# cwitkowitz/amt-tools

Measured on AMD Instinct MI355X. Metric: audio frames/sec (OnsetsFrames+Mel-229 inference), higher is better.
Workload: dtype bf16

## Files before the change

amt_tools_amd/_lib.py:

```python
import ctypes as C
import os
import re

_HERE = os.path.dirname(os.path.abspath(__file__))
LIB_PATH = os.environ.get('AMTX_LIB_PATH') or os.path.join(_HERE, 'csrc', 'libamtx.so')
HEADER_PATH = os.path.join(os.path.dirname(_HERE), 'include', 'amtx.h')

_lib = None


class AmtxError(RuntimeError):
    pass


ERR_UNSUPPORTED = -3


def declared_symbols():
    with open(HEADER_PATH) as f:
        text = f.read()
    text = re.sub(r'/\*.*?\*/', '', text, flags=re.S)
    return sorted(set(re.findall(r'\b(amtx_[a-z0-9_]+)\s*\(', text)))


# ... 11 lines not shown
    'amtx_spec_num_frames': (_L, [_P, _L]),
    'amtx_spec_filterbank': (_I, [_P, _P]),
    'amtx_spec_power': (_I, [_P, _P, _L, _L, _I, _P, _P, _P]),
    'amtx_spec_scale': (_I, [_P, _P, _P, _P, _I, _L, _I, _I, _P, _P]),
    'amtx_of_model_create': (_I, [C.POINTER(_P), _I, _I, _I, _I, _I, _I]),
    'amtx_has_f16': (_I, []),
    'amtx_of_model_destroy': (_I, [_P]),
    'amtx_of_model_set_tensor': (_I, [_P, C.c_char_p, _P, _L]),
    'amtx_of_model_finalize': (_I, [_P]),
    'amtx_of_model_set_tensor_device': (_I, [_P, C.c_char_p, _P, _L]),
    'amtx_of_model_finalize_device': (_I, [_P, _P]),
    'amtx_of_workspace_bytes': (C.c_size_t, [_P, _I, _I]),
    'amtx_of_forward': (_I, [_P, _P, _L, _L, _L, _L, _I, _I, _P, C.c_size_t, _P, _P, _P, _P, _P, _P]),
    'amtx_of_fuses_db_scale': (_I, [_P]),
    'amtx_of_conv_stack_fused': (_I, [_P, _I, _I]),
    'amtx_of_forward_power': (_I, [_P, _P, _L, _L, _L, _P, _P, _I, _I, _P, C.c_size_t, _P, _P, _P, _P, _P, _P]),
    'amtx_of_takes_feats16': (_I, [_P]),
    'amtx_of_forward_feats16': (_I, [_P, _P, _I, _I, _P, C.c_size_t, _P, _P, _P, _P, _P, _P]),
    'amtx_of_offsets': (_I, [_P, _P, C.c_size_t, _I, _I, _P, _P, _P]),
    'amtx_of_num_stages': (_I, []),
    'amtx_of_stage_name': (C.c_char_p, [_I]),
    'amtx_of_profile_enable': (_I, [_P, _I]),
    'amtx_of_profile_read': (_I, [_P, C.POINTER(C.c_double), C.POINTER(_I)]),
    'amtx_linear_packed_elems': (_L, [_I, _I, _I]),
    'amtx_linear_pack': (_I, [_P, _I, _I, _I, _P]),
    'amtx_linear_fwd': (_I, [_P, _L, _I, _P, _I, _P, _P, _L, _I, _L, _I, _I, _P]),
    'amtx_split_planes': (_I, [_P, _L, _I, _P, _I, _L, _L, _P]),
    'amtx_linear_fwd_split': (_I, [_P, _L, _L, _P, _P, _P, _L, _I, _L, _L, _I, _I, _P]),
    'amtx_conv3x3_packed_elems': (_L, [_I, _I]),
    'amtx_conv3x3_pack': (_I, [_P, _P, _I, _I, _P]),
# ... 130 lines not shown
```

amt_tools_amd/csrc/amtx_f16_names.h:

```cpp
#pragma once
#ifdef AMTX_F16
#define amtx_conv3x3_wfrag_elems amtx_conv3x3_wfrag_elems_f16
#define amtx_conv3x3_pack_host amtx_conv3x3_pack_host_f16
#define amtx_conv1_wfrag_elems amtx_conv1_wfrag_elems_f16
#define amtx_conv1_pack_host amtx_conv1_pack_host_f16
#define amtx_launch_conv3x3 amtx_launch_conv3x3_f16
#define amtx_launch_conv1 amtx_launch_conv1_f16
#define amtxdbg_conv_prof amtxdbg_conv_prof_f16
#define amtx_conv_stack_fused_ok amtx_conv_stack_fused_ok_f16
#define amtx_launch_conv_stack amtx_launch_conv_stack_f16
#define amtxdbg_convf_prof amtxdbg_convf_prof_f16
#define amtx_conv3x3_gen_ntc amtx_conv3x3_gen_ntc_f16
#define amtx_conv3x3_gen_wfrag_elems amtx_conv3x3_gen_wfrag_elems_f16
#define amtx_conv3x3_gen_pack_host amtx_conv3x3_gen_pack_host_f16
#define amtx_conv1g_wfrag_elems amtx_conv1g_wfrag_elems_f16
#define amtx_conv1g_pack_host amtx_conv1g_pack_host_f16
#define amtx_conv3x3_gen_can_fuse1 amtx_conv3x3_gen_can_fuse1_f16
#define amtx_launch_conv3x3_gen amtx_launch_conv3x3_gen_f16
#define amtxdbg_convg_prof amtxdbg_convg_prof_f16
#define amtx_pack_bn_fold_dev amtx_pack_bn_fold_dev_f16
#define amtx_pack_conv3x3_dev amtx_pack_conv3x3_dev_f16
#define amtx_pack_conv1_dev amtx_pack_conv1_dev_f16
#define amtx_pack_conv_gen_dev amtx_pack_conv_gen_dev_f16
#define amtx_pack_conv1g_dev amtx_pack_conv1g_dev_f16
#define amtx_pack_scale_rows_dev amtx_pack_scale_rows_dev_f16
// ... 19 lines not shown
```

amt_tools_amd/csrc/amtx_kernels.h:

```cpp
#pragma once
#include "amtx_common.h"

enum { AMTX_T_BF16 = 0, AMTX_T_F32 = 1, AMTX_T_SPLIT = 2 };

static inline size_t amtx_tsize(int t) { return t == AMTX_T_BF16 ? 2 : 4; }

struct GemmArgs {
    const void* A; int64_t lda; int a_type;
    const bf16_t* W; int n_pad, k_pad, planes;
    const float* bias;
    void* C; int64_t ldc; int c_type;
    int64_t M; int N, K;
    int groups; int64_t a_gs, w_gs, bias_gs, c_gs;
    const int2* pair_map = nullptr; float* pair_out = nullptr; int64_t pair_gs = 0, pair_pitch = 0;
    int pair_rows[16] = {0, 0, 0, 0, 0, 0, 0, 0, 0, 0, 0, 0, 0, 0, 0, 0};
    float* pair_max = nullptr; int pair_nh = 0;
    float* roll_out = nullptr; int roll_T = 0; float roll_thr = 0.5f; int roll_group = 0;
    bf16_t* copy16 = nullptr; int64_t copy16_ld = 0; int copy16_col0 = 0, copy16_gs = 0, copy16_pad = 0;
    int64_t a_plane = 0;
    int64_t a_valid_lo = 0, a_valid_hi = 0;
    int64_t a_split = 0, c_split = 0;
};
bool amtx_gemm_has_roll_epilogue(const GemmArgs& g);
int amtx_launch_gemm(const GemmArgs& g, hipStream_t stream);
// ... 3 lines not shown
void amtx_gemm_pack_dims(int N, int K, int* n_pad, int* k_pad);
void amtx_gemm_pack_host(const float* W, int64_t ldw, int N, int K, int planes, bf16_t* out);

struct ConvArgs {
    const void* in; int in_type;
    const bf16_t* wfrag; int planes;
    const float* shift;
    void* out; int out_type;
    int B, T, F, c_out;
    int groups; int64_t in_gs, w_gs, shift_gs, out_gs;
    const float* feats = nullptr; int64_t f_stride_b = 0, f_stride_c = 0, f_stride_t = 0, f_stride_f = 0;
    int c_in = 0;
    const bf16_t* w1frag = nullptr; const float* shift1 = nullptr;
    int64_t w1_gs = 0;
    const float* f_clip_max = nullptr; const float* f_ref = nullptr;
    const void* feats16 = nullptr;
    int64_t out_ts = 0;
    int64_t in_split = 0, out_split = 0;
};
int amtx_launch_conv3x3(const ConvArgs& c, hipStream_t stream);
int amtx_launch_convx3(const ConvArgs& c, hipStream_t stream);
int amtx_launch_convx12(const ConvArgs& c, hipStream_t stream);
size_t amtx_conv1_wfrag_elems(int c_in, int planes);
void amtx_conv1_pack_host(const float* w, const float* scale, int c_in, int planes, bf16_t* out);
size_t amtx_conv3x3_wfrag_elems(int c_out, int planes);
void amtx_conv3x3_pack_host(const float* w, const float* scale, int c_out, int planes, bf16_t* out);

bool amtx_conv_stack_fused_ok(int B, int T, int F, int groups);
int amtx_launch_conv_stack(const ConvArgs& c2, const bf16_t* w3frag, int64_t w3_gs, const float* shift3, void* out, int64_t out_gs,
                           int64_t out_plane, hipStream_t stream);

int amtx_conv3x3_gen_ntc(int c_in, int c_out);
size_t amtx_conv3x3_gen_wfrag_elems(int c_in, int c_out, int planes);
void amtx_conv3x3_gen_pack_host(const float* w , const float* scale, int c_in, int c_out, int planes, bf16_t* out);
int amtx_launch_conv3x3_gen(const ConvArgs& c, int c_in, hipStream_t stream);
static inline __host__ __device__ bool amtx_conv1g_tapk(int c_in, int planes) { return (planes == 1 || planes == 2) && c_in >= 2 && c_in <= 8; }
size_t amtx_conv1g_wfrag_elems(int c_in, int c_mid, int planes);
void amtx_conv1g_pack_host(const float* w , const float* scale, int c_in, int c_mid, int planes, bf16_t* out);
bool amtx_conv3x3_gen_can_fuse1(int c_in, int c_mid, int c_out, int planes);

struct Conv1Args {
    const float* in; int64_t stride_b, stride_c, stride_t, stride_f;
    const float* w;
// ... 59 lines not shown
```

amt_tools_amd/csrc/convf.hip:

```cpp

#include "amtx_f16_names.h"
#include "amtx_kernels.h"

#include <algorithm>
#include <cstdlib>

namespace {

constexpr int RT = 4;
constexpr int R2 = 16 * RT;
constexpr int r3_of(bool halo) { return halo ? R2 - 2 : R2 - 4; }
constexpr int r1_of(bool halo) { return halo ? R2 + 2 : R2; }
constexpr int R1A = R2 + 2;
constexpr int RFA = R1A + 2;
constexpr int CS = 8;
constexpr int CP = CS / 2;
constexpr int RC1 = 2 * CS + 2;
constexpr int RC2 = 2 * CP + 2;
constexpr int PITCH1 = RC1 + 1;
constexpr int PITCH2 = RC2 + 1;
constexpr int ROWB1 = PITCH1 * 16, ROWB2 = PITCH2 * 16;
constexpr int PLANE1 = (R1A * ROWB1 + 255) / 256 * 256;
constexpr int PLANE2 = (R2 * ROWB2 + 255) / 256 * 256;
constexpr int A1_OFF = 0;
constexpr int A2_OFF = 4 * PLANE1;
constexpr int SLAB_COLS = CS + 4;
constexpr int SLAB_LOAD = CS + 2;
constexpr int SLABP = SLAB_COLS * 2;
constexpr int SLAB_BYTES = (RFA * SLABP + 15) / 16 * 16;
constexpr int SLAB_OFF = A2_OFF + 4 * PLANE2;
constexpr int SH3_OFF = SLAB_OFF + 3 * SLAB_BYTES + 128 + 1024;
constexpr int W1_OFF = SH3_OFF + 64 * 4;
constexpr int SH1_OFF = W1_OFF + 8 * 1024;
constexpr int LDS_BYTES = SH1_OFF + 32 * 4;
constexpr int FPRE = (RFA * SLAB_LOAD + 255) / 256;
constexpr int XB = CS / 4;
static_assert(LDS_BYTES <= 160 * 1024, "LDS");
static_assert(CP == 4 && XB == 2, "wave roles below are written for 8 layer2 columns per step");

typedef __attribute__((ext_vector_type(8))) __bf16 mfma_bf16x8;
__device__ __forceinline__ f32x4_t mfma16(uint4 a, uint4 b, f32x4_t c) {
    return amtx_mfma_16x16x32(a, b, c);
}
__device__ __forceinline__ void settle(const uint4& v) { asm volatile("" ::"v"(v.x), "v"(v.y), "v"(v.z), "v"(v.w)); }
__device__ __forceinline__ void settle(float v) { asm volatile("" ::"v"(v)); }

#ifdef AMTX_CONVF_TIMING
__device__ unsigned long long g_convf_prof[16];
#define CONVF_TICK(SLOT)                                                   \
    do {                                                                   \
        const unsigned long long now_ = __builtin_readcyclecounter();      \
        prof_acc[SLOT] += now_ - prof_t;                                   \
        prof_t = now_;                                                     \
    } while (0)
#else
#define CONVF_TICK(SLOT) do {} while (0)
#endif
#if defined(AMTX_CONVF_TIMING) || defined(AMTX_CONVF_ABLATE)
#define CONVF_DBG(BIT) ((dbg & (BIT)) != 0)
#else
#define CONVF_DBG(BIT) false
#endif

struct ConvFArgs {
    const float* feats; int64_t f_stride_b, f_stride_t, f_stride_f;
    const float* f_clip_max; const float* f_ref;
    const bf16_t* w1frag; int64_t w1_gs; const float* shift1;
    const bf16_t* w2frag; int64_t w2_gs; const float* shift2;
    const bf16_t* w3frag; int64_t w3_gs; const float* shift3;
    bf16_t* out; int64_t out_gs;
    int64_t out_plane;
    int B, T, F;
};

struct Pos { int kk, j, b, r0; };
template <int R3_>
__device__ __forceinline__ Pos pos_first_t(int first, int ntt) {
    Pos p;
    p.kk = 0; p.j = 0; p.b = first / ntt; p.r0 = (first - p.b * ntt) * R3_;
    return p;
}
template <int R3_>
__device__ __forceinline__ void pos_next_t(Pos& p, int nstep, int ntt) {
    ++p.kk;
    if (++p.j == nstep) {
        p.j = 0;
        p.r0 += R3_;
        if (p.r0 >= ntt * R3_) { p.r0 = 0; ++p.b; }
    }
}

template <bool HALO>
__global__ __launch_bounds__(512, 2) void convf_kernel(ConvFArgs a, int nstep, int ntt, int nstrips, int per_block, int dbg) {
    constexpr int R3 = r3_of(HALO), R1 = r1_of(HALO), RF = R1 + 2;
    constexpr int FITEMS = RF * SLAB_LOAD;
    constexpr int NUNITS = RT * XB + (HALO ? 1 : 0);
    auto pos_first = [](int first_, int ntt_) { return pos_first_t<R3>(first_, ntt_); };
    auto pos_next = [](Pos& p_, int nstep_, int ntt_) { pos_next_t<R3>(p_, nstep_, ntt_); };
    extern __shared__ __attribute__((aligned(16))) char smem[];
    const int tid = threadIdx.x, lane = tid & 63;
    const int wave = __builtin_amdgcn_readfirstlane(tid >> 6);
    const int grp = blockIdx.y;
    const int g = lane >> 4, trow = lane & 15;
    const int first = blockIdx.x * per_block;
    const int mine = min(per_block, nstrips - first);
    if (mine <= 0) return;
    const int K = mine * nstep;
    const int F2 = a.F >> 1, F4 = F2 >> 1;
    const bool db = a.f_clip_max != nullptr;

    typedef short s16x2 __attribute__((ext_vector_type(2)));
#define CONVF_L1_BEGIN(P, U)                                                                                \
        const char* slab = smem + SLAB_OFF + ((P).kk & 1) * SLAB_BYTES;                                     \
        const int base1 = ((P).kk * CS) % RC1;       \
        const int u = (U);                                                                                  \
        const bool mainu = !HALO || u < NUNITS - 1;                                             \
        const int row1 = mainu ? 16 * (u >> 1) + n16 : R2 + (n16 & 1);                                      \
        const int xb = mainu ? (u & 1) : (n16 >> 1);                                                        \
        const char* fp = slab + (row1 + gg) * SLABP + 8 * xb;                                               \
        const uint2 b0 = *reinterpret_cast<const uint2*>(fp);                                               \
        const uint2 b1 = *reinterpret_cast<const uint2*>(fp + 8);                                           \
        const uint4 bh = make_uint4(b0.x, b0.y, b1.x, b1.y);                                                \
         \
            \
        const uint32_t rowmask = ((unsigned)((P).r0 - 2 + row1) < (unsigned)a.T && xb < XB) ? 0xffffffffu : 0u; \
        const int c1l = CS * (P).j - 1 + 4 * xb;                 \
        const int slotl = base1 + 4 * xb;                                                                   \
        const int dst_row = A1_OFF + g1 * PLANE1 + row1 * ROWB1;                                            \
        const int dst_scratch = SLAB_OFF + 2 * SLAB_BYTES + 128 + (lane_o & 63) * 16;                       \
         \
            \
        const int tu_ = (P).r0 - 2 + 16 * (u >> 1), cu_ = CS * (P).j - 1 + 4 * (u & 1);                     \
        const bool lean = mainu && tu_ >= 0 && tu_ + 15 < a.T && cu_ >= 0 && cu_ + 3 < a.F;                 \
        const int slots_ = base1 + 4 * (u & 1);
#define CONVF_L1_STORE_LEAN(Q, ACC0, ACC1)                                                                  \
        do {                                                                                                \
            uint32_t pk[4];                                                                                 \
            pk[0] = pack_bf16x2((ACC0)[0], (ACC0)[1]); pk[1] = pack_bf16x2((ACC0)[2], (ACC0)[3]);           \
            pk[2] = pack_bf16x2((ACC1)[0], (ACC1)[1]); pk[3] = pack_bf16x2((ACC1)[2], (ACC1)[3]);           \
            _Pragma("unroll") for (int h = 0; h < 4; ++h)                                                   \
                pk[h] = __builtin_bit_cast(uint32_t, __builtin_elementwise_max(__builtin_bit_cast(s16x2, pk[h]), (s16x2){0, 0})); \
            int sq = slots_ + (Q);                                                                          \
            sq = sq >= RC1 ? sq - RC1 : sq;                                                                 \
            *reinterpret_cast<uint4*>(smem + dst_row + sq * 16) = make_uint4(pk[0], pk[1], pk[2], pk[3]);   \
// ... 41 lines not shown
                for (int nt = 0; nt < 2; ++nt) settle(w1t[q][nt]);
#pragma unroll
            for (int tap = 0; tap < 9; ++tap)
#pragma unroll
                for (int nt = 0; nt < 2; ++nt) settle(wf[tap][nt]);
#pragma unroll
            for (int nt = 0; nt < 2; ++nt)
#pragma unroll
                for (int r = 0; r < 4; ++r) { settle(sh1[nt][r]); settle(sh2[nt][r]); }
        }
        if constexpr (!HALO) {
            constexpr int per = (R1A - R1) * ROWB1 / 16;
            for (int i = tid; i < 4 * per; i += 256)
                reinterpret_cast<uint4*>(smem + A1_OFF + (i / per) * PLANE1 + R1 * ROWB1)[i % per] = make_uint4(0, 0, 0, 0);
        }
        for (int i = tid; i < 2 * RFA * 2; i += 256) {
            const int s = i / (RFA * 2), r = i % (RFA * 2);
            *reinterpret_cast<uint16_t*>(smem + SLAB_OFF + s * SLAB_BYTES + (r >> 1) * SLABP + (SLAB_LOAD + (r & 1)) * 2) = 0;
        }

        float fpre[FPRE];
        float fown = 0.f, fref = 0.f;
        unsigned fvalid = 0;
        int fcell[FPRE], foff[FPRE], loff[FPRE];
#pragma unroll
        for (int n = 0; n < FPRE; ++n) {
            const int it = tid + 256 * n;
            const int fi = it / SLAB_LOAD, fc = it % SLAB_LOAD;
            fcell[n] = it < FITEMS ? (fi << 8 | fc) : -256;
            foff[n] = it < FITEMS ? fi * (int)a.f_stride_t + fc * (int)a.f_stride_f : 0;
            loff[n] = it < FITEMS ? fi * SLABP + fc * 2 : 2 * SLAB_BYTES + 64 + (tid & 31) * 2;
        }
        const int fst = (int)a.f_stride_t, fsf = (int)a.f_stride_f;
#define CONVF_ISSUE_LOADS(P)                                                                                \
        do {                                                                                                \
            const float* fb = a.feats + (int64_t)(P).b * a.f_stride_b;                                      \
            const int tb = (P).r0 - 3, cb = CS * (P).j - 2;                                                 \
            const int wb = tb * fst + cb * fsf;                  \
            fvalid = 0;                                                                                     \
            _Pragma("unroll") for (int n = 0; n < FPRE; ++n) {                                              \
                const bool ok = (unsigned)(tb + (fcell[n] >> 8)) < (unsigned)a.T && (unsigned)(cb + (fcell[n] & 255)) < (unsigned)a.F; \
                fvalid |= ok ? (1u << n) : 0u;                                                              \
                fpre[n] = fb[(unsigned)(ok ? wb + foff[n] : 0)];                                            \
            }                                                                                               \
            if (db) {    \
                fown = a.f_clip_max[(P).b];                                                                 \
                fref = a.f_ref[(P).b];                                                                      \
            }                                                                                               \
        } while (0)
#define CONVF_WRITE_SLAB(KK)                                                                                \
        do {                                                                                                \
            DbScale dbs = {0.f, 0.f};                                                                       \
            if (db) dbs = db_scale_make(fown, fref);                                                        \
            char* slab = smem + SLAB_OFF + ((KK) & 1) * SLAB_BYTES;                                         \
            _Pragma("unroll") for (int n = 0; n < FPRE; ++n) {                                              \
                float v = fpre[n];                                                                          \
                if (db) v = db_scale_apply(v, dbs);                                                         \
                v = (fvalid >> n) & 1u ? v : 0.f;                                                           \
                *reinterpret_cast<uint16_t*>(slab + loff[n]) = (uint16_t)pack_bf16x2(v, 0.f);               \
            }                                                                                               \
        } while (0)

        const int lane_a2 = A2_OFF + g * PLANE2 + trow * ROWB2;
        const int n16 = trow, g1 = g, gg = min(g, 2), lane_o = lane;
        const int lane_a1 = A1_OFF + g * PLANE1 + trow * ROWB1;
#define CONVF_L1_PUNIT(P, U)                                                                                \
        do {                                                                                                \
            CONVF_L1_BEGIN(P, U)                                                                            \
            f32x4_t acc1[4][2];                                                                             \
            _Pragma("unroll") for (int q = 0; q < 4; ++q)                                                   \
                _Pragma("unroll") for (int nt = 0; nt < 2; ++nt) acc1[q][nt] = mfma16(w1t[q][nt], bh, sh1[nt]); \
            if (lean) {                                                                                     \
                _Pragma("unroll") for (int q = 0; q < 4; ++q) CONVF_L1_STORE_LEAN(q, acc1[q][0], acc1[q][1]); \
            } else {                                                                                        \
                _Pragma("unroll") for (int q = 0; q < 4; ++q) CONVF_L1_STORE(q, acc1[q][0], acc1[q][1]);    \
            }                                                                                               \
        } while (0)
#define CONVF_L1_PRODUCER(P)                                                                                \
        do {                                                                                                \
            CONVF_L1_PUNIT(P, wave);                                                                        \
            if (HALO && ((P).kk & 3) == wave) CONVF_L1_PUNIT(P, NUNITS - 1);                                \
        } while (0)

        Pos pl = pos_first(first, ntt), p1 = pl, p0 = pl;
        CONVF_ISSUE_LOADS(pl);
        CONVF_WRITE_SLAB(0);
        pos_next(pl, nstep, ntt);
        if (K > 1) {
            CONVF_ISSUE_LOADS(pl);
            CONVF_WRITE_SLAB(1);
            pos_next(pl, nstep, ntt);
        }
        if (K > 2) {
            CONVF_ISSUE_LOADS(pl);
            pos_next(pl, nstep, ntt);
        }
        __syncthreads();
        CONVF_L1_PRODUCER(p1);
        pos_next(p1, nstep, ntt);
        lds_only_barrier();

#ifdef AMTX_CONVF_TIMING
        unsigned long long prof_acc[4] = {0, 0, 0, 0};
        unsigned long long prof_t = __builtin_readcyclecounter();
#endif
        __builtin_amdgcn_s_setprio(2);
        for (int kk = 0; kk <= K; ++kk) {
            if (kk < K) {
                if (!CONVF_DBG(2)) {
                    const int base1 = (p0.kk * CS) % RC1;
                    const int base2 = (p0.kk * CP) % RC2;
                    const int p = CP * p0.j - 1 + wave;
                    const bool pvalid = p >= 0 && p < F2;
                    int addr[4];
#pragma unroll
                    for (int cc = 0; cc < 4; ++cc) addr[cc] = lane_a1 + ((base1 + RC1 + 2 * wave - 2 + cc) % RC1) * 16;
                    int slot2 = base2 + wave;
                    slot2 = slot2 >= RC2 ? slot2 - RC2 : slot2;
                    char* dst2 = smem + lane_a2 + slot2 * 16;
                    const int nrt = pvalid ? min(RT, (a.T - p0.r0 + 16) >> 4) : 0;
                    uint4 x[3][4];
#define CONVF_LOAD_ROW2(KH, RTI)                                                                            \
                    _Pragma("unroll") for (int cc = 0; cc < 4; ++cc)                                        \
// ... 34 lines not shown
                            for (int nt = 0; nt < 2; ++nt)
#pragma unroll
                                for (int r = 0; r < 4; ++r) v[nt * 4 + r] = fmaxf(fmaxf(acc[0][nt][r], acc[1][nt][r]), 0.f);
                            const int t2 = p0.r0 - 1 + 16 * rt + trow;
                            const uint32_t rowmask = (unsigned)t2 < (unsigned)a.T ? 0xffffffffu : 0u;
                            o = make_uint4(pack_bf16x2(v[0], v[1]) & rowmask, pack_bf16x2(v[2], v[3]) & rowmask,
                                           pack_bf16x2(v[4], v[5]) & rowmask, pack_bf16x2(v[6], v[7]) & rowmask);
                        }
                        *reinterpret_cast<uint4*>(dst2 + (16 * rt) * ROWB2) = o;
                    }
#undef CONVF_LOAD_ROW2
                }
                pos_next(p0, nstep, ntt);
                CONVF_TICK(0);
                __builtin_amdgcn_s_setprio(3);
                if (!CONVF_DBG(8)) {
                    if (kk + 2 < K) CONVF_WRITE_SLAB(kk + 2);
                    if (kk + 3 < K) {
                        CONVF_ISSUE_LOADS(pl);
                        pos_next(pl, nstep, ntt);
                    }
                }
                if (kk + 1 < K) {
                    if (!CONVF_DBG(1)) CONVF_L1_PRODUCER(p1);
                    pos_next(p1, nstep, ntt);
                }
                __builtin_amdgcn_s_setprio(2);
                CONVF_TICK(1);
            }
            lds_only_barrier();
            CONVF_TICK(2);
        }
#ifdef AMTX_CONVF_TIMING
        if (tid == 0) {
            for (int i = 0; i < 3; ++i) atomicAdd(&g_convf_prof[i], prof_acc[i]);
            atomicAdd(&g_convf_prof[3], (unsigned long long)(K + 1));
        }
#endif
#undef CONVF_ISSUE_LOADS
#undef CONVF_WRITE_SLAB
#undef CONVF_L1_PRODUCER
#undef CONVF_L1_PUNIT
    } else {
        uint4 wf[9][4];
        {
            const int gr = (lane & 15) >> 2;
#pragma unroll
            for (int nt = 0; nt < 4; ++nt) {
                const int src_lane = (lane & 48) + 4 * (2 * (nt >> 1) + (gr >> 1)) + (lane & 3);
                const uint4* w = reinterpret_cast<const uint4*>(a.w3frag + (int64_t)grp * a.w3_gs) + src_lane;
#pragma unroll
                for (int tap = 0; tap < 9; ++tap) wf[tap][nt] = w[(tap * 4 + 2 * (gr & 1) + (nt & 1)) * 64];
            }
#pragma unroll
            for (int tap = 0; tap < 9; ++tap)
#pragma unroll
// ... 19 lines not shown
                _Pragma("unroll") for (int nt = 0; nt < 2; ++nt) w1l[q][nt] = *reinterpret_cast<const uint4*>(wl + (2 * q + nt) * 1024); \
            f32x4_t acc1[4][2];                                                                             \
            _Pragma("unroll") for (int q = 0; q < 4; ++q)                                                   \
                _Pragma("unroll") for (int nt = 0; nt < 2; ++nt) acc1[q][nt] = mfma16(w1l[q][nt], bh, sh1l[nt]); \
            if (lean) {                                                                                     \
                _Pragma("unroll") for (int q = 0; q < 4; ++q) CONVF_L1_STORE_LEAN(q, acc1[q][0], acc1[q][1]); \
            } else {                                                                                        \
                _Pragma("unroll") for (int q = 0; q < 4; ++q) CONVF_L1_STORE(q, acc1[q][0], acc1[q][1]);    \
            }                                                                                               \
        } while (0)
#define CONVF_L1_CONSUMER(P)                                                                                \
        do {                                                                                                \
            CONVF_L1_CUNIT(P, wave);                                                                        \
        } while (0)
        Pos pc1 = pos_first(first, ntt);
        CONVF_L1_CONSUMER(pc1);
        pos_next(pc1, nstep, ntt);
        lds_only_barrier();

        const int mi = (wave - 4) & 1;
        const int rt0 = ((wave - 4) >> 1) * 2;
        const int lane_a2 = A2_OFF + g * PLANE2 + (16 * rt0 + trow) * ROWB2;
        Pos pc = pos_first(first, ntt);
#ifdef AMTX_CONVF_TIMING
        unsigned long long prof_acc[4] = {0, 0, 0, 0};
        unsigned long long prof_t = __builtin_readcyclecounter();
#endif
        for (int kk = 0; kk <= K; ++kk) {
            if (kk + 1 < K) {
                __builtin_amdgcn_s_setprio(3);
                if (!CONVF_DBG(1)) CONVF_L1_CONSUMER(pc1);
                __builtin_amdgcn_s_setprio(0);
                pos_next(pc1, nstep, ntt);
            }
            CONVF_TICK(0);
            if (kk >= 1) {
                if (!CONVF_DBG(4)) {
                    const int base2 = (pc.kk * CP) % RC2;
                    const int m = (CP / 2) * pc.j - 1 + mi;
                    const bool mvalid = m >= 0 && m < F4;
                    const int nrt = mvalid ? min(2, (a.T - pc.r0 + 15 - 16 * rt0) >> 4) : 0;
                    int addr[4];
#pragma unroll
                    for (int cc = 0; cc < 4; ++cc) addr[cc] = lane_a2 + ((base2 + RC2 + 2 * mi - 2 + cc) % RC2) * 16;
// ... 59 lines not shown
#undef CONVF_L1_CUNIT
#undef CONVF_L1_CONSUMER
#ifdef AMTX_CONVF_TIMING
        if (tid == 256) {
            for (int i = 0; i < 3; ++i) atomicAdd(&g_convf_prof[8 + i], prof_acc[i]);
            atomicAdd(&g_convf_prof[11], (unsigned long long)(K + 1));
        }
#endif
    }
}

#undef CONVF_L1_BEGIN
#undef CONVF_L1_STORE
#undef CONVF_L1_STORE_LEAN

}

static int convf_steps(int F) {
    const int F4 = (F >> 1) >> 1;
    int n = 1;
    while (2 * (n - 1) < F4 - 1) ++n;
    return n;
}

static bool convf_halo(int T) { return (T + r3_of(true) - 1) / r3_of(true) < (T + r3_of(false) - 1) / r3_of(false); }

bool amtx_conv_stack_fused_ok(int B, int T, int F, int groups) {
    if (F < 4 || B <= 0 || T <= 0 || groups <= 0) return false;
    const int r3 = r3_of(convf_halo(T));
    const int64_t strips = (int64_t)B * ((T + r3 - 1) / r3) * groups;
    return strips >= 256 && (int64_t)B * ((T + r3 - 1) / r3) < (1ll << 30);
}

int amtx_launch_conv_stack(const ConvArgs& c2, const bf16_t* w3frag, int64_t w3_gs, const float* shift3, void* out, int64_t out_gs,
                           int64_t out_plane, hipStream_t stream) {
    AMTX_REQUIRE(c2.feats && c2.c_in == 1 && c2.w1frag && c2.shift1 && c2.wfrag && c2.shift && w3frag && shift3 && out,
                 "conv_stack: null pointer / not a one-channel input");
    AMTX_REQUIRE(c2.planes == 1 && c2.c_out == 32 && c2.out_type == AMTX_T_BF16, "conv_stack: bf16, 32 -> 32 -> 64 channels only");
    AMTX_REQUIRE(c2.B > 0 && c2.T > 0 && c2.F >= 4 && c2.groups > 0, "conv_stack: bad sizes");
    AMTX_REQUIRE(c2.f_stride_t >= 0 && c2.f_stride_f >= 0 && (int64_t)c2.T * c2.f_stride_t + (int64_t)c2.F * c2.f_stride_f < (1ll << 31),
                 "conv_stack: a clip's feature view must span fewer than 2^31 elements with non-negative strides");
    ConvFArgs a;
    a.feats = c2.feats; a.f_stride_b = c2.f_stride_b; a.f_stride_t = c2.f_stride_t; a.f_stride_f = c2.f_stride_f;
    a.f_clip_max = c2.f_clip_max; a.f_ref = c2.f_ref ? c2.f_ref : c2.f_clip_max;
    a.w1frag = c2.w1frag; a.w1_gs = c2.w1_gs; a.shift1 = c2.shift1;
    a.w2frag = c2.wfrag; a.w2_gs = c2.w_gs; a.shift2 = c2.shift;
    a.w3frag = w3frag; a.w3_gs = w3_gs; a.shift3 = shift3;
    a.out = (bf16_t*)out; a.out_gs = out_gs; a.out_plane = out_plane;
    a.B = c2.B; a.T = c2.T; a.F = c2.F;
    const bool halo = convf_halo(c2.T);
    const int r3 = r3_of(halo);
    const int ntt = (c2.T + r3 - 1) / r3;
    const int64_t nstrips = (int64_t)c2.B * ntt;
    AMTX_REQUIRE(nstrips < (1ll << 30), "conv_stack: grid too large");
    const int nstep = convf_steps(c2.F);
    AMTX_REQUIRE((int64_t)nstep * (nstrips + 1) < (1ll << 31), "conv_stack: too many steps");
    int gx = std::max(1, 256 / c2.groups);
    if (gx > nstrips) gx = (int)nstrips;
    const int per_block = (int)((nstrips + gx - 1) / gx);
    gx = (int)((nstrips + per_block - 1) / per_block);
    auto kern = halo ? convf_kernel<true> : convf_kernel<false>;
    AMTX_GRANT_LDS(convf_kernel<true>, LDS_BYTES);
    AMTX_GRANT_LDS(convf_kernel<false>, LDS_BYTES);
    int dbg = 0;
#if defined(AMTX_CONVF_TIMING) || defined(AMTX_CONVF_ABLATE)
    if (const char* e = getenv("AMTX_CONVF_DBG")) dbg = atoi(e);
#endif
    hipLaunchKernelGGL(kern, dim3((unsigned)gx, (unsigned)c2.groups), dim3(512), LDS_BYTES, stream, a, nstep, ntt, (int)nstrips, per_block, dbg);
    AMTX_CHECK_LAUNCH();
    return AMTX_OK;
}

#ifdef AMTX_CONVF_TIMING
extern "C" int amtxdbg_convf_prof(unsigned long long* out16, int reset) {
    if (hipMemcpyFromSymbol(out16, HIP_SYMBOL(g_convf_prof), 16 * sizeof(unsigned long long)) != hipSuccess) return -1;
    if (reset) {
        unsigned long long z[16] = {0};
        if (hipMemcpyToSymbol(HIP_SYMBOL(g_convf_prof), z, sizeof(z)) != hipSuccess) return -1;
// ... 5 lines not shown
```

amt_tools_amd/csrc/ofmodel.hip:

```cpp

#include "amtx_kernels.h"
#include "amtx_kernels_f16.h"

#include <cmath>
#include <cstdlib>
#include <map>
#include <string>
#include <thread>
#include <vector>

namespace {

struct Tensor { std::vector<float> v; };

inline size_t align256(size_t x) { return (x + 255) & ~(size_t)255; }

struct DevBuf {
    void* p = nullptr;
    size_t bytes = 0;
    int upload(const void* host, size_t n) {
        if (!p || bytes != n) {
            if (p) (void)hipFree(p);
            p = nullptr; bytes = n;
            AMTX_CHECK_HIP(hipMalloc(&p, n));
// ... 126 lines not shown
}

struct Workspace {
    char *a1, *a2, *a3, *e, *xp, *l1, *joint, *joint16, *xp2, *l2, *mp;
    size_t total;
};

Workspace carve(const amtx_of_model* m, int B, int T, char* base) {
    Workspace w;
    const size_t es = amtx_tsize(m->act_type);
    const size_t BT = (size_t)B * T;
    const int F = m->dim_in, F2 = F / 2;
    size_t off = 0;
    auto take = [&](size_t bytes) { char* p = base ? base + off : nullptr; off += align256(bytes); return p; };
    w.a1 = take(m->fuse_conv1 ? 256 : BT * F * m->nf1 * es * m->n_heads);
    w.a2 = take(m->fuse_stack && amtx_conv_stack_fused_ok(B, T, F, m->n_heads) ? 256 : BT * F2 * m->nf2 * es * m->n_heads);
    w.a3 = take(BT * m->kfc_pad * es * m->n_heads);
    w.e = take(BT * m->dim_am * es * m->n_heads);
    w.xp = take(BT * m->xw * es * m->n_rec);
    w.l1 = take(BT * m->dim_lm * es * m->n_rec);
    w.joint = take(BT * m->dim_aj * sizeof(float));
    w.joint16 = take(BT * (size_t)((m->dim_aj + 63) / 64 * 64) * 2 * (m->split_acts ? 2 : 1));
    w.xp2 = take(BT * m->xw * es);
    w.l2 = take(BT * m->dim_lm * es);
    w.mp = take(BT * m->n_out * sizeof(float));
    w.total = off;
    return w;
}

}

// ... 468 lines not shown
        c2.c_in = m->in_channels; c2.w1frag = (const bf16_t*)m->conv1_frag.p; c2.shift1 = (const float*)m->conv1_s.p;
        c2.w1_gs = (int64_t)(m->gen_conv2 ? amtx_conv1g_wfrag_elems(m->in_channels, m->nf1, pl) : amtx_conv1_wfrag_elems(m->in_channels, pl));
        c2.f_clip_max = clip_max; c2.f_ref = ref;
        if (feats16) { c2.feats = nullptr; c2.feats16 = feats16; }
    }
    const bool x12m_now = feats16 && m->x12m;
    if (x12m_now) {
        c2.in_split = BT * F * 8;
        c2.wfrag = (const bf16_t*)m->conv2_wx.p;
        c2.w_gs = (int64_t)amtx_conv3x3_wfrag_elems(m->nf2, pl);
    }
    const bool fused_stack = m->fuse_stack && amtx_conv_stack_fused_ok(B, T, F, m->n_heads);
    static const bool rowmajor_a3 = getenv("AMTX_OF_ROWMAJOR_A3") != nullptr;
    const int64_t a3_plane = (fused_stack && !rowmajor_a3 && m->nf3 == 64 && m->kfc_pad == m->kfc) ? BT * 64 : 0;
    if (fused_stack) {
        if ((rc = (f16 ? amtx_launch_conv_stack_f16 : amtx_launch_conv_stack)(c2, (const bf16_t*)m->conv3_w.p, (int64_t)amtx_conv3x3_wfrag_elems(m->nf3, pl), (const float*)m->conv3_s.p,
                                         w.a3, BT * m->kfc_pad, a3_plane, s)) != AMTX_OK) return rc;
    } else if (x12m_now) {
        if ((rc = amtx_launch_convx12(c2, s)) != AMTX_OK) return rc;
    } else if ((rc = m->gen_conv2 ? launch_convg(c2, m->nf1, s) : launch_conv(c2, s)) != AMTX_OK) return rc;
    mark();

    ConvArgs c3 = c2;
    c3.feats = nullptr; c3.feats16 = nullptr; c3.w1frag = nullptr; c3.shift1 = nullptr; c3.c_in = 0;
    c3.in = w.a2; c3.wfrag = (const bf16_t*)m->conv3_w.p; c3.shift = (const float*)m->conv3_s.p; c3.out = w.a3;
    c3.F = F2; c3.c_out = m->nf3; c3.in_gs = BT * F2 * m->nf2;
    c3.w_gs = (int64_t)(m->gen_conv ? amtx_conv3x3_gen_wfrag_elems(m->nf2, m->nf3, pl) : amtx_conv3x3_wfrag_elems(m->nf3, pl));
    c3.shift_gs = m->nf3; c3.out_gs = BT * m->kfc_pad;
    if (sp) { c3.in_type = AMTX_T_SPLIT; c3.in_split = a2_split; c3.out_type = AMTX_T_SPLIT; c3.out_split = a3_split; }
    if (m->kfc_pad != m->kfc) {
// ... 171 lines not shown
```

include/amtx.h:

```cpp
#ifndef AMTX_H
#define AMTX_H

#include <stddef.h>
#include <stdint.h>

#ifdef __cplusplus
extern "C" {
#endif

#define AMTX_OK 0
#define AMTX_ERR_ARG (-1)
#define AMTX_ERR_HIP (-2)
#define AMTX_ERR_UNSUPPORTED (-3)

#define AMTX_PREC_BF16 0
#define AMTX_PREC_X3 1
#define AMTX_PREC_F16 2

const char* amtx_last_error(void);
int amtx_version(void);

typedef struct amtx_spec_plan amtx_spec_plan;

#define AMTX_PAD_CONSTANT 0
// ... 35 lines not shown
int amtx_of_fuses_db_scale(const amtx_of_model* model);
int amtx_of_forward_power(const amtx_of_model* model, const float* power, int64_t stride_b, int64_t stride_t, int64_t stride_f,
                          const float* clip_max, const float* ref, int batch, int num_frames, void* workspace, size_t workspace_bytes,
                          float* out_onsets, float* out_multi_pitch, float* logits_onsets, float* logits_multi_pitch,
                          float* logits_pitch_head, void* stream);

int amtx_of_takes_feats16(const amtx_of_model* model);
int amtx_of_forward_feats16(const amtx_of_model* model, const void* feats16, int batch, int num_frames, void* workspace, size_t workspace_bytes,
                            float* out_onsets, float* out_multi_pitch, float* logits_onsets, float* logits_multi_pitch,
                            float* logits_pitch_head, void* stream);

int amtx_of_model_set_tensor_device(amtx_of_model* model, const char* name, const float* device_data, int64_t numel);
int amtx_of_model_finalize_device(amtx_of_model* model, void* stream);

int amtx_of_conv_stack_fused(const amtx_of_model* model, int batch, int num_frames);

int amtx_of_offsets(const amtx_of_model* model, void* workspace, size_t workspace_bytes, int batch, int num_frames, float* out_offsets,
                    float* logits_offsets, void* stream);

int amtx_of_num_stages(void);
const char* amtx_of_stage_name(int stage);
int amtx_of_profile_enable(amtx_of_model* model, int enable);
int amtx_of_profile_read(amtx_of_model* model, double* stage_ms , int* num_forwards);

int64_t amtx_linear_packed_elems(int n, int k, int planes);
int amtx_linear_pack(const float* host_w, int n, int k, int planes, uint16_t* host_out);
int amtx_linear_fwd(const void* a, int64_t lda, int a_type, const uint16_t* w_packed, int planes, const float* bias, void* c,
                    int64_t ldc, int c_type, int64_t m, int n, int k, void* stream);
int amtx_split_planes(const float* src, int64_t ld_src, int n, uint16_t* dst, int ld_dst, int64_t split, int64_t rows, void* stream);
int amtx_linear_fwd_split(const void* a, int64_t lda, int64_t a_split, const uint16_t* w_packed, const float* bias, void* c, int64_t ldc,
// ... 106 lines not shown
```

Measured before the change: 40.79 million.

## Prebuild dB-scaled bf16 slab map and DMA slabs into LDS for fused conv stack

Adds a pre-pass kernel that applies the dB scale to raw power and writes it as bf16 slabs laid out in the fused conv kernel's LDS format, one per strip step. The fused conv kernel gets a MAP variant that loads these slabs straight into a triple-buffered LDS ring with global-to-LDS DMA instead of register loads, scaling and LDS writes. Its layer-1 producer then computes both column halves per wave, and the separate consumer layer-1 path is dropped. The cost is an extra kernel launch, a workspace map sized to the input, and extra global traffic for the map, in exchange for less in-loop work and register pressure.

```diff
diff --git a/amt_tools_amd/_lib.py b/amt_tools_amd/_lib.py
--- a/amt_tools_amd/_lib.py
+++ b/amt_tools_amd/_lib.py
@@ -49,6 +49,7 @@
     'amtx_of_forward': (_I, [_P, _P, _L, _L, _L, _L, _I, _I, _P, C.c_size_t, _P, _P, _P, _P, _P, _P]),
     'amtx_of_fuses_db_scale': (_I, [_P]),
     'amtx_of_conv_stack_fused': (_I, [_P, _I, _I]),
+    'amtx_conv_stack_slab_map': (_I, [_P, _L, _L, _L, _P, _P, _I, _I, _I, _P, _P]),
     'amtx_of_forward_power': (_I, [_P, _P, _L, _L, _L, _P, _P, _I, _I, _P, C.c_size_t, _P, _P, _P, _P, _P, _P]),
     'amtx_of_takes_feats16': (_I, [_P]),
     'amtx_of_forward_feats16': (_I, [_P, _P, _I, _I, _P, C.c_size_t, _P, _P, _P, _P, _P, _P]),
diff --git a/amt_tools_amd/csrc/amtx_f16_names.h b/amt_tools_amd/csrc/amtx_f16_names.h
--- a/amt_tools_amd/csrc/amtx_f16_names.h
+++ b/amt_tools_amd/csrc/amtx_f16_names.h
@@ -9,6 +9,8 @@
 #define amtxdbg_conv_prof amtxdbg_conv_prof_f16
 #define amtx_conv_stack_fused_ok amtx_conv_stack_fused_ok_f16
 #define amtx_launch_conv_stack amtx_launch_conv_stack_f16
+#define amtx_conv_stack_slab_bytes amtx_conv_stack_slab_bytes_f16
+#define amtx_conv_stack_slab_map amtx_conv_stack_slab_map_f16
 #define amtxdbg_convf_prof amtxdbg_convf_prof_f16
 #define amtx_conv3x3_gen_ntc amtx_conv3x3_gen_ntc_f16
 #define amtx_conv3x3_gen_wfrag_elems amtx_conv3x3_gen_wfrag_elems_f16
diff --git a/amt_tools_amd/csrc/amtx_kernels.h b/amt_tools_amd/csrc/amtx_kernels.h
--- a/amt_tools_amd/csrc/amtx_kernels.h
+++ b/amt_tools_amd/csrc/amtx_kernels.h
@@ -41,6 +41,7 @@
     const bf16_t* w1frag = nullptr; const float* shift1 = nullptr;
     int64_t w1_gs = 0;
     const float* f_clip_max = nullptr; const float* f_ref = nullptr;
+    void* f_slabs = nullptr;
     const void* feats16 = nullptr;
     int64_t out_ts = 0;
     int64_t in_split = 0, out_split = 0;
@@ -54,6 +55,7 @@
 void amtx_conv3x3_pack_host(const float* w, const float* scale, int c_out, int planes, bf16_t* out);
 
 bool amtx_conv_stack_fused_ok(int B, int T, int F, int groups);
+size_t amtx_conv_stack_slab_bytes(int B, int T, int F);
 int amtx_launch_conv_stack(const ConvArgs& c2, const bf16_t* w3frag, int64_t w3_gs, const float* shift3, void* out, int64_t out_gs,
                            int64_t out_plane, hipStream_t stream);
 
diff --git a/amt_tools_amd/csrc/convf.hip b/amt_tools_amd/csrc/convf.hip
--- a/amt_tools_amd/csrc/convf.hip
+++ b/amt_tools_amd/csrc/convf.hip
@@ -27,15 +27,18 @@
 constexpr int SLAB_COLS = CS + 4;
 constexpr int SLAB_LOAD = CS + 2;
 constexpr int SLABP = SLAB_COLS * 2;
-constexpr int SLAB_BYTES = (RFA * SLABP + 15) / 16 * 16;
+constexpr int SLAB_CHUNKS = RFA * SLABP / 16;
+constexpr int SLAB_STRIDE = 2048;
 constexpr int SLAB_OFF = A2_OFF + 4 * PLANE2;
-constexpr int SH3_OFF = SLAB_OFF + 3 * SLAB_BYTES + 128 + 1024;
+constexpr int SCR_OFF = SLAB_OFF + 3 * SLAB_STRIDE + 128;
+constexpr int SH3_OFF = SCR_OFF + 1024;
 constexpr int W1_OFF = SH3_OFF + 64 * 4;
 constexpr int SH1_OFF = W1_OFF + 8 * 1024;
 constexpr int LDS_BYTES = SH1_OFF + 32 * 4;
 constexpr int FPRE = (RFA * SLAB_LOAD + 255) / 256;
 constexpr int XB = CS / 4;
 static_assert(LDS_BYTES <= 160 * 1024, "LDS");
+static_assert(RFA * SLABP % 16 == 0 && 2 * 64 >= SLAB_CHUNKS && SLAB_STRIDE >= 2 * 64 * 16, "a slab is two 64-lane 16-byte DMA instructions");
 static_assert(CP == 4 && XB == 2, "wave roles below are written for 8 layer2 columns per step");
 
 typedef __attribute__((ext_vector_type(8))) __bf16 mfma_bf16x8;
@@ -65,6 +68,7 @@
 struct ConvFArgs {
     const float* feats; int64_t f_stride_b, f_stride_t, f_stride_f;
     const float* f_clip_max; const float* f_ref;
+    const char* slabs; int64_t slab_clip, slab_step;
     const bf16_t* w1frag; int64_t w1_gs; const float* shift1;
     const bf16_t* w2frag; int64_t w2_gs; const float* shift2;
     const bf16_t* w3frag; int64_t w3_gs; const float* shift3;
@@ -90,7 +94,7 @@
     }
 }
 
-template <bool HALO>
+template <bool HALO, bool MAP>
 __global__ __launch_bounds__(512, 2) void convf_kernel(ConvFArgs a, int nstep, int ntt, int nstrips, int per_block, int dbg) {
     constexpr int R3 = r3_of(HALO), R1 = r1_of(HALO), RF = R1 + 2;
     constexpr int FITEMS = RF * SLAB_LOAD;
@@ -111,7 +115,7 @@
 
     typedef short s16x2 __attribute__((ext_vector_type(2)));
 #define CONVF_L1_BEGIN(P, U)                                                                                \
-        const char* slab = smem + SLAB_OFF + ((P).kk & 1) * SLAB_BYTES;                                     \
+        const char* slab = smem + SLAB_OFF + (MAP ? (P).kk % 3 : (P).kk & 1) * SLAB_STRIDE;                  \
         const int base1 = ((P).kk * CS) % RC1;       \
         const int u = (U);                                                                                  \
         const bool mainu = !HALO || u < NUNITS - 1;                                             \
@@ -127,7 +131,7 @@
         const int c1l = CS * (P).j - 1 + 4 * xb;                 \
         const int slotl = base1 + 4 * xb;                                                                   \
         const int dst_row = A1_OFF + g1 * PLANE1 + row1 * ROWB1;                                            \
-        const int dst_scratch = SLAB_OFF + 2 * SLAB_BYTES + 128 + (lane_o & 63) * 16;                       \
+        const int dst_scratch = SCR_OFF + (lane_o & 63) * 16;                                               \
          \
             \
         const int tu_ = (P).r0 - 2 + 16 * (u >> 1), cu_ = CS * (P).j - 1 + 4 * (u & 1);                     \
@@ -199,9 +203,9 @@
             for (int i = tid; i < 4 * per; i += 256)
                 reinterpret_cast<uint4*>(smem + A1_OFF + (i / per) * PLANE1 + R1 * ROWB1)[i % per] = make_uint4(0, 0, 0, 0);
         }
-        for (int i = tid; i < 2 * RFA * 2; i += 256) {
+        if constexpr (!MAP) for (int i = tid; i < 2 * RFA * 2; i += 256) {
             const int s = i / (RFA * 2), r = i % (RFA * 2);
-            *reinterpret_cast<uint16_t*>(smem + SLAB_OFF + s * SLAB_BYTES + (r >> 1) * SLABP + (SLAB_LOAD + (r & 1)) * 2) = 0;
+            *reinterpret_cast<uint16_t*>(smem + SLAB_OFF + s * SLAB_STRIDE + (r >> 1) * SLABP + (SLAB_LOAD + (r & 1)) * 2) = 0;
         }
 
         float fpre[FPRE];
@@ -214,7 +218,7 @@
             const int fi = it / SLAB_LOAD, fc = it % SLAB_LOAD;
             fcell[n] = it < FITEMS ? (fi << 8 | fc) : -256;
             foff[n] = it < FITEMS ? fi * (int)a.f_stride_t + fc * (int)a.f_stride_f : 0;
-            loff[n] = it < FITEMS ? fi * SLABP + fc * 2 : 2 * SLAB_BYTES + 64 + (tid & 31) * 2;
+            loff[n] = it < FITEMS ? fi * SLABP + fc * 2 : 2 * SLAB_STRIDE + 64 + (tid & 31) * 2;
         }
         const int fst = (int)a.f_stride_t, fsf = (int)a.f_stride_f;
 #define CONVF_ISSUE_LOADS(P)                                                                                \
@@ -237,7 +241,7 @@
         do {                                                                                                \
             DbScale dbs = {0.f, 0.f};                                                                       \
             if (db) dbs = db_scale_make(fown, fref);                                                        \
-            char* slab = smem + SLAB_OFF + ((KK) & 1) * SLAB_BYTES;                                         \
+            char* slab = smem + SLAB_OFF + ((KK) & 1) * SLAB_STRIDE;                                        \
             _Pragma("unroll") for (int n = 0; n < FPRE; ++n) {                                              \
                 float v = fpre[n];                                                                          \
                 if (db) v = db_scale_apply(v, dbs);                                                         \
@@ -261,24 +265,82 @@
                 _Pragma("unroll") for (int q = 0; q < 4; ++q) CONVF_L1_STORE(q, acc1[q][0], acc1[q][1]);    \
             }                                                                                               \
         } while (0)
+#define CONVF_L1_PAIR(P)                                                                                    \
+        do {                                                                                                \
+            const char* slab = smem + SLAB_OFF + ((P).kk % 3) * SLAB_STRIDE;                                \
+            const int base1 = ((P).kk * CS) % RC1;                                                          \
+            const int row1 = 16 * wave + n16;                                                               \
+            const char* fp = slab + (row1 + gg) * SLABP;                                                    \
+            const uint2 b0 = *reinterpret_cast<const uint2*>(fp);                                           \
+            const uint2 b1 = *reinterpret_cast<const uint2*>(fp + 8);                                       \
+            const uint2 b2 = *reinterpret_cast<const uint2*>(fp + 16);                                      \
+            const uint4 bh[2] = {make_uint4(b0.x, b0.y, b1.x, b1.y), make_uint4(b1.x, b1.y, b2.x, b2.y)};   \
+            f32x4_t acc1[2][4][2];                                                                          \
+            _Pragma("unroll") for (int xb = 0; xb < 2; ++xb)                                                \
+                _Pragma("unroll") for (int q = 0; q < 4; ++q)                                               \
+                    _Pragma("unroll") for (int nt = 0; nt < 2; ++nt) acc1[xb][q][nt] = mfma16(w1t[q][nt], bh[xb], sh1[nt]); \
+            const uint32_t rowmask = (unsigned)((P).r0 - 2 + row1) < (unsigned)a.T ? 0xffffffffu : 0u;      \
+            const int dst_row = lane_a1 + 16 * wave * ROWB1;                                                \
+            const int tu_ = (P).r0 - 2 + 16 * wave;                                                         \
+            _Pragma("unroll") for (int xb = 0; xb < 2; ++xb) {                                              \
+                const int c1l = CS * (P).j - 1 + 4 * xb;            \
+                const int slots_ = base1 + 4 * xb;                                                          \
+                if (tu_ >= 0 && tu_ + 15 < a.T && c1l >= 0 && c1l + 3 < a.F) {                             \
+                    _Pragma("unroll") for (int q = 0; q < 4; ++q) CONVF_L1_STORE_LEAN(q, acc1[xb][q][0], acc1[xb][q][1]); \
+                } else {                                                                                    \
+                    _Pragma("unroll") for (int q = 0; q < 4; ++q) {                                         \
+                        uint32_t pk[4];                                                                     \
+                        pk[0] = pack_bf16x2(acc1[xb][q][0][0], acc1[xb][q][0][1]); pk[1] = pack_bf16x2(acc1[xb][q][0][2], acc1[xb][q][0][3]); \
+                        pk[2] = pack_bf16x2(acc1[xb][q][1][0], acc1[xb][q][1][1]); pk[3] = pack_bf16x2(acc1[xb][q][1][2], acc1[xb][q][1][3]); \
+                        const uint32_t keep = (unsigned)(c1l + q) < (unsigned)a.F ? rowmask : 0u;          \
+                        _Pragma("unroll") for (int h = 0; h < 4; ++h)                                       \
+                            pk[h] = __builtin_bit_cast(uint32_t, __builtin_elementwise_max(__builtin_bit_cast(s16x2, pk[h]), (s16x2){0, 0})) & keep; \
+                        int sq = slots_ + q;                                                                \
+                        sq = sq >= RC1 ? sq - RC1 : sq;                                                     \
+                        *reinterpret_cast<uint4*>(smem + dst_row + sq * 16) = make_uint4(pk[0], pk[1], pk[2], pk[3]); \
+                    }                                                                                       \
+                }                                                                                           \
+            }                                                                                               \
+        } while (0)
 #define CONVF_L1_PRODUCER(P)                                                                                \
         do {                                                                                                \
-            CONVF_L1_PUNIT(P, wave);                                                                        \
+            if constexpr (MAP) CONVF_L1_PAIR(P); else CONVF_L1_PUNIT(P, wave);                              \
             if (HALO && ((P).kk & 3) == wave) CONVF_L1_PUNIT(P, NUNITS - 1);                                \
         } while (0)
+        const unsigned lds_slabs = __builtin_amdgcn_readfirstlane((unsigned)(uintptr_t)(lds_void_t*)smem) + SLAB_OFF;
+#define CONVF_SLAB_DMA(P)                                                                                   \
+        do {                                                                                                \
+            if (wave < 2)                                                                                   \
+                glds16(a.slabs + (P).b * a.slab_clip + (P).j * a.slab_step + (int64_t)(P).r0 * SLABP + min(64 * wave + lane, SLAB_CHUNKS - 1) * 16, \
+                       lds_slabs + ((P).kk % 3) * SLAB_STRIDE + wave * 1024);                               \
+        } while (0)
 
         Pos pl = pos_first(first, ntt), p1 = pl, p0 = pl;
-        CONVF_ISSUE_LOADS(pl);
-        CONVF_WRITE_SLAB(0);
-        pos_next(pl, nstep, ntt);
-        if (K > 1) {
+        if constexpr (MAP) {
+            CONVF_SLAB_DMA(pl);
+            pos_next(pl, nstep, ntt);
+            if (K > 1) {
+                CONVF_SLAB_DMA(pl);
+                pos_next(pl, nstep, ntt);
+            }
+            wait_vm<0>();
+            if (K > 2) {
+                CONVF_SLAB_DMA(pl);
+                pos_next(pl, nstep, ntt);
+            }
+        } else {
             CONVF_ISSUE_LOADS(pl);
-            CONVF_WRITE_SLAB(1);
+            CONVF_WRITE_SLAB(0);
             pos_next(pl, nstep, ntt);
-        }
-        if (K > 2) {
-            CONVF_ISSUE_LOADS(pl);
-            pos_next(pl, nstep, ntt);
+            if (K > 1) {
+                CONVF_ISSUE_LOADS(pl);
+                CONVF_WRITE_SLAB(1);
+                pos_next(pl, nstep, ntt);
+            }
+            if (K > 2) {
+                CONVF_ISSUE_LOADS(pl);
+                pos_next(pl, nstep, ntt);
+            }
         }
         __syncthreads();
         CONVF_L1_PRODUCER(p1);
@@ -292,6 +354,12 @@
         __builtin_amdgcn_s_setprio(2);
         for (int kk = 0; kk <= K; ++kk) {
             if (kk < K) {
+                if constexpr (MAP) {
+                    if (kk + 3 < K) {
+                        CONVF_SLAB_DMA(pl);
+                        pos_next(pl, nstep, ntt);
+                    }
+                }
                 if (!CONVF_DBG(2)) {
                     const int base1 = (p0.kk * CS) % RC1;
                     const int base2 = (p0.kk * CP) % RC2;
@@ -356,7 +424,7 @@
                 pos_next(p0, nstep, ntt);
                 CONVF_TICK(0);
                 __builtin_amdgcn_s_setprio(3);
-                if (!CONVF_DBG(8)) {
+                if (!MAP && !CONVF_DBG(8)) {
                     if (kk + 2 < K) CONVF_WRITE_SLAB(kk + 2);
                     if (kk + 3 < K) {
                         CONVF_ISSUE_LOADS(pl);
@@ -370,6 +438,9 @@
                 __builtin_amdgcn_s_setprio(2);
                 CONVF_TICK(1);
             }
+            if constexpr (MAP) {
+                if (kk + 3 < K) wait_vm<1>(); else wait_vm<0>();
+            }
             lds_only_barrier();
             CONVF_TICK(2);
         }
@@ -382,6 +453,8 @@
 #undef CONVF_ISSUE_LOADS
 #undef CONVF_WRITE_SLAB
 #undef CONVF_L1_PRODUCER
+#undef CONVF_L1_PAIR
+#undef CONVF_SLAB_DMA
 #undef CONVF_L1_PUNIT
     } else {
         uint4 wf[9][4];
@@ -431,7 +504,7 @@
             CONVF_L1_CUNIT(P, wave);                                                                        \
         } while (0)
         Pos pc1 = pos_first(first, ntt);
-        CONVF_L1_CONSUMER(pc1);
+        if constexpr (!MAP) CONVF_L1_CONSUMER(pc1);
         pos_next(pc1, nstep, ntt);
         lds_only_barrier();
 
@@ -444,7 +517,7 @@
         unsigned long long prof_t = __builtin_readcyclecounter();
 #endif
         for (int kk = 0; kk <= K; ++kk) {
-            if (kk + 1 < K) {
+            if (!MAP && kk + 1 < K) {
                 __builtin_amdgcn_s_setprio(3);
                 if (!CONVF_DBG(1)) CONVF_L1_CONSUMER(pc1);
                 __builtin_amdgcn_s_setprio(0);
@@ -534,6 +607,48 @@
 #undef CONVF_L1_STORE
 #undef CONVF_L1_STORE_LEAN
 
+constexpr int MAP_RB = 32;
+constexpr int SLAB_TAIL = 2048;
+constexpr int MAP_WC = 272;
+__global__ __launch_bounds__(256) void convf_slab_map_kernel(const float* __restrict__ pw, int64_t sb, int64_t st, int64_t sf,
+                                                             const float* __restrict__ clip_max, const float* __restrict__ ref,
+                                                             char* __restrict__ map, int T, int F, int nstep, int TP) {
+    __shared__ __attribute__((aligned(16))) uint16_t row[MAP_RB][MAP_WC];
+    const int wc = CS * nstep + 4;
+    const int b = blockIdx.y, m0 = blockIdx.x * MAP_RB;
+    const DbScale dbs = db_scale_make(clip_max[b], ref[b]);
+    const float* pb = pw + (int64_t)b * sb;
+    for (int c = threadIdx.x; c < wc; c += 256) {
+        const int f = c - 2;
+        const bool fok = (unsigned)f < (unsigned)F;
+#pragma unroll 4
+        for (int r = 0; r < MAP_RB; ++r) {
+            const int t = m0 + r - 3;
+            float v = 0.f;
+            if (fok && (unsigned)t < (unsigned)T) v = db_scale_apply(pb[t * st + f * sf], dbs);
+            row[r][c] = (uint16_t)pack_bf16x2(v, 0.f);
+        }
+    }
+    __syncthreads();
+    const int nr = min(MAP_RB, TP - m0);
+    const int npc = nr * 24 / 16;
+    for (int i = threadIdx.x; i < nstep * (MAP_RB * 24 / 16); i += 256) {
+        const int j = i / (MAP_RB * 24 / 16), k = i - j * (MAP_RB * 24 / 16);
+        if (k >= npc) continue;
+        uint32_t d[4];
+#pragma unroll
+        for (int h = 0; h < 4; ++h) {
+            const int e = 4 * k + h, r = e / 6, q = e - r * 6;
+            const uint16_t* src = &row[r][CS * j + 2 * q];
+            d[h] = q < 5 ? (src[0] | (uint32_t)src[1] << 16) : 0u;
+        }
+        *reinterpret_cast<uint4*>(map + (((int64_t)b * nstep + j) * TP + m0) * SLABP + k * 16) = make_uint4(d[0], d[1], d[2], d[3]);
+    }
+    if (blockIdx.x == gridDim.x - 1 && b == (int)gridDim.y - 1)
+        for (int i = threadIdx.x; i < SLAB_TAIL / 16; i += 256)
+            reinterpret_cast<uint4*>(map + (int64_t)gridDim.y * nstep * TP * SLABP)[i] = make_uint4(0, 0, 0, 0);
+}
+
 }
 
 static int convf_steps(int F) {
@@ -544,6 +659,29 @@
 }
 
 static bool convf_halo(int T) { return (T + r3_of(true) - 1) / r3_of(true) < (T + r3_of(false) - 1) / r3_of(false); }
+
+static int convf_map_rows(int T) { return (T + 7) & ~1; }
+
+size_t amtx_conv_stack_slab_bytes(int B, int T, int F) {
+    return (size_t)B * convf_steps(F) * convf_map_rows(T) * SLABP + SLAB_TAIL;
+}
+
+static int launch_slab_map(const float* pw, int64_t sb, int64_t st, int64_t sf, const float* clip_max, const float* ref, int B, int T, int F,
+                           void* map, hipStream_t stream) {
+    const int nstep = convf_steps(F), TP = convf_map_rows(T);
+    AMTX_REQUIRE(pw && clip_max && map && B > 0 && T > 0 && F >= 4, "conv_stack: slab map: null pointer / bad sizes");
+    AMTX_REQUIRE(CS * nstep + 4 <= MAP_WC && ((uintptr_t)map & 15) == 0,
+                 "conv_stack: a slab map needs at most 264 frequency bins and a 16-byte aligned workspace");
+    hipLaunchKernelGGL(convf_slab_map_kernel, dim3((unsigned)((TP + MAP_RB - 1) / MAP_RB), (unsigned)B), dim3(256), 0, stream,
+                       pw, sb, st, sf, clip_max, ref ? ref : clip_max, (char*)map, T, F, nstep, TP);
+    AMTX_CHECK_LAUNCH();
+    return AMTX_OK;
+}
+
+extern "C" int amtx_conv_stack_slab_map(const float* power, int64_t stride_b, int64_t stride_t, int64_t stride_f, const float* clip_max,
+                                        const float* ref, int batch, int num_frames, int dim_in, void* map, void* stream) {
+    return launch_slab_map(power, stride_b, stride_t, stride_f, clip_max, ref, batch, num_frames, dim_in, map, (hipStream_t)stream);
+}
 
 bool amtx_conv_stack_fused_ok(int B, int T, int F, int groups) {
     if (F < 4 || B <= 0 || T <= 0 || groups <= 0) return false;
@@ -563,6 +701,7 @@
     ConvFArgs a;
     a.feats = c2.feats; a.f_stride_b = c2.f_stride_b; a.f_stride_t = c2.f_stride_t; a.f_stride_f = c2.f_stride_f;
     a.f_clip_max = c2.f_clip_max; a.f_ref = c2.f_ref ? c2.f_ref : c2.f_clip_max;
+    const bool map = c2.f_clip_max && c2.f_slabs;
     a.w1frag = c2.w1frag; a.w1_gs = c2.w1_gs; a.shift1 = c2.shift1;
     a.w2frag = c2.wfrag; a.w2_gs = c2.w_gs; a.shift2 = c2.shift;
     a.w3frag = w3frag; a.w3_gs = w3_gs; a.shift3 = shift3;
@@ -579,9 +718,17 @@
     if (gx > nstrips) gx = (int)nstrips;
     const int per_block = (int)((nstrips + gx - 1) / gx);
     gx = (int)((nstrips + per_block - 1) / per_block);
-    auto kern = halo ? convf_kernel<true> : convf_kernel<false>;
-    AMTX_GRANT_LDS(convf_kernel<true>, LDS_BYTES);
-    AMTX_GRANT_LDS(convf_kernel<false>, LDS_BYTES);
+    AMTX_REQUIRE(!c2.f_slabs || c2.f_clip_max, "conv_stack: a slab map is made of raw power");
+    a.slabs = (const char*)c2.f_slabs; a.slab_step = (int64_t)convf_map_rows(c2.T) * SLABP; a.slab_clip = a.slab_step * nstep;
+    int rc;
+    if (map && (rc = launch_slab_map(c2.feats, c2.f_stride_b, c2.f_stride_t, c2.f_stride_f, a.f_clip_max, a.f_ref, c2.B, c2.T, c2.F,
+                                     c2.f_slabs, stream)) != AMTX_OK)
+        return rc;
+    auto kern = map ? (halo ? convf_kernel<true, true> : convf_kernel<false, true>) : (halo ? convf_kernel<true, false> : convf_kernel<false, false>);
+    AMTX_GRANT_LDS((convf_kernel<true, false>), LDS_BYTES);
+    AMTX_GRANT_LDS((convf_kernel<false, false>), LDS_BYTES);
+    AMTX_GRANT_LDS((convf_kernel<true, true>), LDS_BYTES);
+    AMTX_GRANT_LDS((convf_kernel<false, true>), LDS_BYTES);
     int dbg = 0;
 #if defined(AMTX_CONVF_TIMING) || defined(AMTX_CONVF_ABLATE)
     if (const char* e = getenv("AMTX_CONVF_DBG")) dbg = atoi(e);
diff --git a/amt_tools_amd/csrc/ofmodel.hip b/amt_tools_amd/csrc/ofmodel.hip
--- a/amt_tools_amd/csrc/ofmodel.hip
+++ b/amt_tools_amd/csrc/ofmodel.hip
@@ -164,7 +164,9 @@
     size_t off = 0;
     auto take = [&](size_t bytes) { char* p = base ? base + off : nullptr; off += align256(bytes); return p; };
     w.a1 = take(m->fuse_conv1 ? 256 : BT * F * m->nf1 * es * m->n_heads);
-    w.a2 = take(m->fuse_stack && amtx_conv_stack_fused_ok(B, T, F, m->n_heads) ? 256 : BT * F2 * m->nf2 * es * m->n_heads);
+    const bool fused = m->fuse_stack && amtx_conv_stack_fused_ok(B, T, F, m->n_heads);
+    const bool power = m->fuse_conv1 && !m->gen_conv2 && m->in_channels == 1;
+    w.a2 = take(fused ? (power ? amtx_conv_stack_slab_bytes(B, T, F) : 256) : BT * F2 * m->nf2 * es * m->n_heads);
     w.a3 = take(BT * m->kfc_pad * es * m->n_heads);
     w.e = take(BT * m->dim_am * es * m->n_heads);
     w.xp = take(BT * m->xw * es * m->n_rec);
@@ -663,6 +665,8 @@
     static const bool rowmajor_a3 = getenv("AMTX_OF_ROWMAJOR_A3") != nullptr;
     const int64_t a3_plane = (fused_stack && !rowmajor_a3 && m->nf3 == 64 && m->kfc_pad == m->kfc) ? BT * 64 : 0;
     if (fused_stack) {
+        static const bool raw_staging = getenv("AMTX_CONVF_RAW_STAGING") != nullptr;
+        if (clip_max && !raw_staging) c2.f_slabs = w.a2;
         if ((rc = (f16 ? amtx_launch_conv_stack_f16 : amtx_launch_conv_stack)(c2, (const bf16_t*)m->conv3_w.p, (int64_t)amtx_conv3x3_wfrag_elems(m->nf3, pl), (const float*)m->conv3_s.p,
                                          w.a3, BT * m->kfc_pad, a3_plane, s)) != AMTX_OK) return rc;
     } else if (x12m_now) {
diff --git a/include/amtx.h b/include/amtx.h
--- a/include/amtx.h
+++ b/include/amtx.h
@@ -73,6 +73,9 @@
 int amtx_of_model_finalize_device(amtx_of_model* model, void* stream);
 
 int amtx_of_conv_stack_fused(const amtx_of_model* model, int batch, int num_frames);
+
+int amtx_conv_stack_slab_map(const float* power, int64_t stride_b, int64_t stride_t, int64_t stride_f, const float* clip_max,
+                             const float* ref, int batch, int num_frames, int dim_in, void* map, void* stream);
 
 int amtx_of_offsets(const amtx_of_model* model, void* workspace, size_t workspace_bytes, int batch, int num_frames, float* out_offsets,
                     float* logits_offsets, void* stream);
```

After: 40.70 million (median of 2 runs). No clear change (-0.2%).
